# ppwwyyxx/OpenPano

Measured on NVIDIA H100. Metric: Mpixels/sec SIFT+match+blend, higher is better.
Workload: dtype f32

## Files before the change

openpano_b200/csrc/blend.cu:

```cuda
#include "common.cuh"
#include "blend_rows.cuh"
#include "blur_tile.cuh"
#include <math.h>
#include <string.h>
#include <vector>
#include <algorithm>
#include <climits>
#include <memory>

struct BlendImg {
  union {
    const float* rgb;
    const unsigned char* pix;
  };
  int w, h;
  int x0, y0, x1, y1;
  double hi[9];
  long long roi_off;
  long long plane;
  long long mask_off;
  int rw, rh, pitch;
  int channels;
};

// ... 131 lines not shown
  wsum[t] = ws;
}

__global__ void k_linear_resolve(const float* sum, const float* __restrict__ wsum, float* out, size_t n_px, int lazy) {
  const size_t t = (size_t)blockIdx.x * blockDim.x + threadIdx.x;
  if (t >= n_px) return;
  const float* p = sum + t * 3;
  linear_resolve_px(lazy, p[0], p[1], p[2], wsum[t], out + t * 3);
}

template <class Src>
__global__ void k_mb_first_level(const BlendImg* __restrict__ imgs, BlendGeom g, float* __restrict__ cur,
                                 unsigned char* __restrict__ mask) {
  __shared__ float lut[Src::kLut ? 256 : 1];
  if constexpr (Src::kLut) {
    build_rgb8_lut(lut, threadIdx.y * blockDim.x + threadIdx.x);
    __syncthreads();
  }
  const BlendImg& im = imgs[blockIdx.z];
  int j = blockIdx.x * blockDim.x + threadIdx.x;
  int i = blockIdx.y * blockDim.y + threadIdx.y;
  if (j >= im.rw || i >= im.rh) return;
  double x, y;
  coor_func(im, g, j + im.x0, i + im.y0, &x, &y);
  float c0, c1, c2;
  bool ok = interpolate_rgb(blend_src<Src>(im, lut), im.w, im.h, (float)y, (float)x, &c0, &c1, &c2);
  if (ok && fminf(c0, fminf(c1, c2)) < 0) ok = false;
  const size_t o = (size_t)i * im.pitch + j;
  float* p = cur + im.roi_off + o;
  float ww = 0.f;
  if (!ok) { c0 = 0.f; c1 = 0.f; c2 = 0.f; }
  else {
    double ox = x / im.w - 0.5, oy = y / im.h - 0.5;
    double wd = (0.5 - fabs(ox)) * (0.5 - fabs(oy));
    if (wd < 0.0) wd = 0.0;
    ww = (float)(wd + 1e-6);
  }
  p[0] = c0; p[im.plane] = c1; p[2 * im.plane] = c2; p[3 * im.plane] = ww;
  mask[im.mask_off + o] = ok ? 0 : 1;
}

__global__ void k_mb_weight_argmax(const BlendImg* __restrict__ imgs, int n, float* __restrict__ cur, int tw,
                                   int row0, int row1) {
  __shared__ TileList tl;
  {
    const int tj0 = blockIdx.x * blockDim.x, ti0 = row0 + blockIdx.y * blockDim.y;
    build_tile_list(imgs, n, tj0, ti0, tj0 + blockDim.x - 1, ti0 + blockDim.y - 1, &tl);
  }
  int j = blockIdx.x * blockDim.x + threadIdx.x;
  int i = row0 + blockIdx.y * blockDim.y + threadIdx.y;
  if (j >= tw || i >= row1) return;
  const int nl = tl.n < 0 ? n : tl.n;
  float mx = 0.f;
  int best = -1;
  for (int q = 0; q < nl; ++q) {
    const BlendImg& im = imgs[tl.n < 0 ? q : (int)tl.idx[q]];
    if (i >= im.y0 && i <= im.y1 && j >= im.x0 && j <= im.x1) {
      const float w = __ldg(cur + im.roi_off + 3 * im.plane + (size_t)(i - im.y0) * im.pitch + (j - im.x0));
      if (w > mx) { mx = w; best = q; }
    }
  }
  for (int q = 0; q < nl; ++q) {
    const BlendImg& im = imgs[tl.n < 0 ? q : (int)tl.idx[q]];
    if (i >= im.y0 && i <= im.y1 && j >= im.x0 && j <= im.x1)
      cur[im.roi_off + 3 * im.plane + (size_t)(i - im.y0) * im.pitch + (j - im.x0)] = q == best ? 1.f : 0.f;
  }
}

struct BlurTaps { int center; float taps[64]; };
struct MbPlane { long long off; int w, h, pitch, pad; };

template <int C>
__global__ void __launch_bounds__(BT_THREADS, 4)
k_mb_blur_tma(const MbPlane* __restrict__ planes, const int2* __restrict__ span, int n_planes, int n_tiles,
              const TmaDesc* __restrict__ maps, float* __restrict__ dst, const __grid_constant__ BlurTaps bt) {
  extern __shared__ __align__(128) float smem[];
  __shared__ __align__(8) uint64_t s_bar[2];
  __shared__ BlurTile s_tile[2];
  constexpr int RX = (C + 3) & ~3;
  constexpr int GW = BT_W + 2 * RX, GH = BT_H + 2 * C;
  constexpr int GSZ = (GH * GW + 31) & ~31;
  float* grey0 = smem;
  float* colbuf = smem + 2 * GSZ;
  float* outT = colbuf + BLUR_COLBUF_FLOATS(C);
  const int tid = threadIdx.x;
  constexpr uint32_t tile_bytes = (uint32_t)(GH * GW * sizeof(float));
  int t = blockIdx.x;
  if (tid == 0) {
    sbar_init(sm_u32(&s_bar[0]), 1);
    sbar_init(sm_u32(&s_bar[1]), 1);
    asm volatile("fence.mbarrier_init.release.cluster;" ::: "memory");
    if (t < n_tiles) {
      const BlurTile tl = find_blur_tile(span, n_planes, t);
      s_tile[0] = tl;
      sbar_expect_tx(sm_u32(&s_bar[0]), tile_bytes);
      tma_load_2d(sm_u32(grey0), maps + tl.om, tl.tx * BT_W - RX, tl.ty * BT_H - C, sm_u32(&s_bar[0]));
    }
  }
  __syncthreads();
  for (int it = 0; t < n_tiles; t += gridDim.x, ++it) {
    const int b = it & 1;
    float* grey = grey0 + b * GSZ;
    const BlurTile tl = s_tile[b];
    const MbPlane pl = planes[tl.om];
    const int x0 = tl.tx * BT_W, y0 = tl.ty * BT_H;
    if (tid == 0 && t + (int)gridDim.x < n_tiles) {
      const BlurTile nx = find_blur_tile(span, n_planes, t + gridDim.x);
      s_tile[b ^ 1] = nx;
      asm volatile("fence.proxy.async.shared::cta;" ::: "memory");
      sbar_expect_tx(sm_u32(&s_bar[b ^ 1]), tile_bytes);
      tma_load_2d(sm_u32(grey0 + (b ^ 1) * GSZ), maps + nx.om, nx.tx * BT_W - RX, nx.ty * BT_H - C, sm_u32(&s_bar[b ^ 1]));
    }
    sbar_wait(sm_u32(&s_bar[b]), (uint32_t)(it >> 1) & 1u);
    if (x0 - RX < 0 || y0 - C < 0 || x0 + BT_W + RX > pl.w || y0 + BT_H + C > pl.h) {
      for (int i = tid; i < GH * GW; i += BT_THREADS) {
        const int yy = i / GW, xx = i - yy * GW;
        const int gy = y0 + yy - C, gx = x0 + xx - RX;
        const int cy = min(max(gy, 0), pl.h - 1), cx = min(max(gx, 0), pl.w - 1);
        if (cy != gy || cx != gx) grey[i] = grey[(cy - y0 + C) * GW + (cx - x0 + RX)];
      }
      __syncthreads();
    }
    blur_level<C>(grey, colbuf, outT, bt.taps, C, RX, GW, tid);
    const int tx = tid & (BT_W - 1), ty = tid / BT_W;
    const int gx = x0 + tx;
    float* out = dst + pl.off;
#pragma unroll
    for (int i = 0; i < BT_H / 4; ++i) {
      const int y = ty + 4 * i, gy = y0 + y;
      if (gx < pl.w && gy < pl.h) out[(size_t)gy * pl.pitch + gx] = outT[y * (BT_W + 1) + tx];
    }
    __syncthreads();
  }
}

#define MB_TW 64
#define MB_TH 32
__global__ void __launch_bounds__(256)
k_mb_blur_generic(const MbPlane* __restrict__ planes, const int2* __restrict__ span, int n_planes,
                  const float* __restrict__ src, float* __restrict__ dst, const __grid_constant__ BlurTaps bt) {
  extern __shared__ float mb_smem[];
  const BlurTile tl = find_blur_tile(span, n_planes, blockIdx.x);
  const MbPlane pl = planes[tl.om];
  const int tx0 = tl.tx * MB_TW, ty0 = tl.ty * MB_TH;
  const int c = bt.center, kw = 2 * c + 1;
  const int SW = MB_TW + 2 * c, SH = MB_TH + 2 * c;
  float* tile = mb_smem;
  float* colres = mb_smem + SH * SW;
  const float* base = src + pl.off;
  const int tid = threadIdx.x;
  for (int idx = tid; idx < SH * SW; idx += 256) {
    const int r = idx / SW, q = idx - r * SW;
    const int y = min(max(ty0 - c + r, 0), pl.h - 1), x = min(max(tx0 - c + q, 0), pl.w - 1);
    tile[idx] = __ldg(base + (size_t)y * pl.pitch + x);
  }
  __syncthreads();
  for (int idx = tid; idx < MB_TH * SW; idx += 256) {
    const int i = idx / SW, q = idx - i * SW;
    float acc = 0.f;
    const float* col = tile + i * SW + q;
    for (int k = 0; k < kw; ++k) acc += col[k * SW] * bt.taps[k];
    colres[idx] = acc;
  }
  __syncthreads();
  for (int idx = tid; idx < MB_TH * MB_TW; idx += 256) {
    const int i = idx / MB_TW, j = idx - i * MB_TW;
    if (ty0 + i >= pl.h || tx0 + j >= pl.w) continue;
    float acc = 0.f;
    const float* row = colres + i * SW + j;
    for (int k = 0; k < kw; ++k) acc += row[k] * bt.taps[k];
    dst[pl.off + (size_t)(ty0 + i) * pl.pitch + tx0 + j] = acc;
  }
}

__global__ void k_mb_accumulate(const BlendImg* __restrict__ imgs, int n, const float* __restrict__ cur,
                                const float* __restrict__ next, const unsigned char* __restrict__ mask,
                                int first, int is_last, float* __restrict__ out, unsigned char* __restrict__ tmask, int tw,
                                int row0, int row1) {
  __shared__ TileList tl;
  {
    const int tj0 = blockIdx.x * blockDim.x, ti0 = row0 + blockIdx.y * blockDim.y;
    build_tile_list(imgs, n, tj0, ti0, tj0 + blockDim.x - 1, ti0 + blockDim.y - 1, &tl);
  }
  int j = blockIdx.x * blockDim.x + threadIdx.x;
  int i = row0 + blockIdx.y * blockDim.y + threadIdx.y;
  if (j >= tw || i >= row1) return;
  const int nl = tl.n < 0 ? n : tl.n;
  float s0 = 0.f, s1 = 0.f, s2 = 0.f, wsum = 0.f;
  for (int q = 0; q < nl; ++q) {
    const BlendImg& im = imgs[tl.n < 0 ? q : (int)tl.idx[q]];
    if (!(i >= im.y0 && i <= im.y1 && j >= im.x0 && j <= im.x1)) continue;
    const size_t o = (size_t)(i - im.y0) * im.pitch + (j - im.x0);
    const float w = __ldg(cur + im.roi_off + 3 * im.plane + o);
    if (w <= 0) continue;
    if (mask[im.mask_off + o]) continue;
    const float* pc = cur + im.roi_off + o;
    const float c0 = __ldg(pc), c1 = __ldg(pc + im.plane), c2 = __ldg(pc + 2 * im.plane);
    if (!is_last) {
      const float* pn = next + im.roi_off + o;
      const float n0 = __ldg(pn), n1 = __ldg(pn + im.plane), n2 = __ldg(pn + 2 * im.plane);
      s0 += (c0 - n0) * w; s1 += (c1 - n1) * w; s2 += (c2 - n2) * w;
    } else {
      s0 += c0 * w; s1 += c1 * w; s2 += c2 * w;
    }
    wsum += w;
  }
  size_t t = (size_t)(i - row0) * tw + j;
  float* p = out + t * 3;
  bool touched = first ? false : tmask[t] != 0;
  float v0 = -1.f, v1 = -1.f, v2 = -1.f;
  if (touched) { v0 = p[0]; v1 = p[1]; v2 = p[2]; }
  bool dirty = first != 0;
  if (!((double)wsum < 1e-6)) {
    s0 /= wsum; s1 /= wsum; s2 /= wsum;
    if (!touched) { v0 = s0; v1 = s1; v2 = s2; touched = true; }
    else { v0 += s0; v1 += s1; v2 += s2; }
    dirty = true;
  }
  if (is_last && touched) {
    v0 = v0 < 1.0f ? v0 : 1.0f; v0 = v0 > 0.f ? v0 : 0.f;
    v1 = v1 < 1.0f ? v1 : 1.0f; v1 = v1 > 0.f ? v1 : 0.f;
    v2 = v2 < 1.0f ? v2 : 1.0f; v2 = v2 > 0.f ? v2 : 0.f;
    dirty = true;
  }
  if (dirty) { p[0] = v0; p[1] = v1; p[2] = v2; }
  if (first || touched) tmask[t] = touched ? 1 : 0;
}

__global__ void k_fill(float* __restrict__ p, size_t n, float v) {
  size_t i = (size_t)blockIdx.x * blockDim.x + threadIdx.x;
  if (i < n) p[i] = v;
}


struct BlendJob {
  std::vector<BlendImg> imgs;
  std::vector<int> src;
  BlendGeom g;
  int tw = 0, th = 0;
  long long roi_floats = 0;
  long long mask_bytes = 0;
  int max_rw = 0, max_rh = 0;
  std::vector<BlurTaps> level_taps;
  int halo = 0;
  bool strip = false;
  int clip0 = INT_MIN, clip1 = INT_MAX;
  std::vector<double> tab;
  size_t ncol = 0, nrow = 0;
};

struct BlendDev {
  DevBuf<BlendImg> d_imgs;
  DevBuf<double> d_tab;
  DevBuf<float> d_cur, d_next;
  DevBuf<unsigned char> d_mask, d_tmask;
  DevBuf<MbPlane> d_planes;
  DevBuf<int2> d_span;
  DevBuf<TmaDesc> d_maps;
  std::vector<int> centers;
  int n_planes = 0, n_tiles = 0;
  int wrow0 = 0, wrow1 = 0;
};

template <int C>
static cudaError_t launch_mb_blur_tma(pano_ctx* ctx, int grid, const MbPlane* planes, const int2* span, int n_planes,
                                      int n_tiles, const TmaDesc* maps, float* dst, const BlurTaps& bt) {
  constexpr int RX = (C + 3) & ~3, GW = BT_W + 2 * RX, GH = BT_H + 2 * C, GSZ = (GH * GW + 31) & ~31;
  const size_t smem = (size_t)(2 * GSZ + BLUR_COLBUF_FLOATS(C) + BT_H * (BT_W + 1)) * sizeof(float);
  cudaError_t e = cudaFuncSetAttribute(k_mb_blur_tma<C>, cudaFuncAttributeMaxDynamicSharedMemorySize, (int)smem);
  if (e != cudaSuccess) return e;
  k_mb_blur_tma<C><<<grid, BT_THREADS, smem, ctx->stream>>>(planes, span, n_planes, n_tiles, maps, dst, bt);
  return cudaGetLastError();
}

static int level_taps(int bands, int gauss_window_factor, std::vector<BlurTaps>* taps) {
  int halo = 0;
  for (int level = 0; level + 1 < bands; ++level) {
    float sigma = (float)(sqrt(level * 2 + 1.0) * 4);
    BlurTaps bt;
    memset(&bt, 0, sizeof(bt));
    int kw = host_gauss_kernel(sigma, gauss_window_factor, bt.taps, 63);
    if (kw < 0) return kw;
    bt.center = kw / 2;
    halo += bt.center;
    if (taps) taps->push_back(bt);
  }
  return halo;
}

int blend_halo(int bands, const pano_params* p) { return level_taps(bands, p->gauss_window_factor, nullptr); }

static void strip_clip(int bands, int halo, int oh, int row0, int row1, int* clip0, int* clip1) {
  const bool strip = bands > 0 && (row0 != 0 || row1 != oh);
  *clip0 = (strip && row0 > 0) ? std::max(0, row0 - halo) : INT_MIN;
  *clip1 = (strip && row1 < oh) ? row1 + halo - 1 : INT_MAX;
}

bool blend_strip_reads(const pano_blend_image& im, int bands, int halo, int oh, int row0, int row1) {
  if (row0 == 0 && row1 == oh) return true;
  if (bands == 0) return im.y0 < row1 && im.y1 >= row0;
  int c0, c1;
  strip_clip(bands, halo, oh, row0, row1, &c0, &c1);
  return std::max(im.y0, c0) <= std::min(im.y1, c1);
}

static int blend_plan(pano_ctx* ctx, int n, const pano_blend_image* imgs, const pano_blend_geom* g, int bands,
                      const pano_params* p, int ow, int oh, int row0, int row1, bool need_src, BlendJob* job,
                      const unsigned char* const* pix = nullptr, const int* channels = nullptr, bool tables = true) {
  job->halo = level_taps(bands, p->gauss_window_factor, &job->level_taps);
  if (job->halo < 0) return ctx_fail(ctx, PANO_ERR_INVALID, "blend: gaussian window %d too wide", -job->halo);
  job->strip = bands > 0 && (row0 != 0 || row1 != oh);
  strip_clip(bands, job->halo, oh, row0, row1, &job->clip0, &job->clip1);
  job->imgs.reserve(n);
  for (int k = 0; k < n; ++k) {
    const pano_blend_image& s = imgs[k];
    if ((need_src && !s.rgb_hwc) || s.w < 2 || s.h < 2 || s.x1 < s.x0 || s.y1 < s.y0 || s.x0 < 0 || s.y0 < 0)
      return ctx_fail(ctx, PANO_ERR_INVALID, "blend: image %d has an invalid shape or range", k);
    if (pix && !pix[k]) return ctx_fail(ctx, PANO_ERR_INVALID, "blend: image %d has no pixels", k);
    if (pix)
      if (int rc = pix8_check(ctx, "blend", k, channels[k], pix[k])) return rc;
    job->tw = std::max(job->tw, s.x1); job->th = std::max(job->th, s.y1);
    BlendImg d;
    memset(&d, 0, sizeof(d));
    d.rgb = s.rgb_hwc; d.w = s.w; d.h = s.h;
    if (pix) d.pix = pix[k];
    d.x0 = s.x0; d.x1 = s.x1;
    d.y0 = std::max(s.y0, job->clip0); d.y1 = std::min(s.y1, job->clip1);
    if (d.y0 > d.y1) continue;
    memcpy(d.hi, s.homo_inv, sizeof(d.hi));
    d.rw = d.x1 - d.x0 + 1; d.rh = d.y1 - d.y0 + 1;
    d.pitch = (int)align_up((size_t)d.rw, 32);
    d.plane = (long long)d.pitch * d.rh;
    d.roi_off = job->roi_floats;
    d.mask_off = job->mask_bytes;
    d.channels = pix ? channels[k] : 3;
    job->roi_floats += 4 * d.plane;
    job->mask_bytes += d.plane;
    job->max_rw = std::max(job->max_rw, d.rw); job->max_rh = std::max(job->max_rh, d.rh);
    job->imgs.push_back(d);
    job->src.push_back(k);
  }
  if (job->tw != ow || job->th != oh || ow <= 0 || oh <= 0)
    return ctx_fail(ctx, PANO_ERR_INVALID, "blend: output is %dx%d but target_size is %dx%d", ow, oh, job->tw, job->th);
  if (job->imgs.empty()) return PANO_OK;
  job->ncol = (size_t)job->tw + 2; job->nrow = (size_t)job->th + 2;
  if (tables && g->projection != PANO_PROJ_FLAT) {
    job->tab.resize(2 * job->ncol + job->nrow);
    for (size_t j = 0; j < job->ncol; ++j) {
      double cx = (double)j * g->res_x + g->proj_min_x;
      job->tab[j] = sin(cx); job->tab[job->ncol + j] = cos(cx);
    }
// ... 454 lines not shown
```

openpano_b200/csrc/blur_tile.cuh:

```cuda
#pragma once
#include "common.cuh"

#define BT_W 64
#define BT_H 32
#define BT_THREADS 256

struct BlurTile { int om; int tx, ty; };

__device__ __forceinline__ BlurTile find_blur_tile(const int2* __restrict__ span, int n_om, int cta) {
  int lo = 0, hi = n_om - 1;
  while (lo < hi) {
    const int mid = (lo + hi + 1) >> 1;
    if (span[mid].x <= cta) lo = mid; else hi = mid - 1;
  }
  const int local = cta - span[lo].x, tx_n = span[lo].y;
  BlurTile t;
  t.om = lo; t.ty = local / tx_n; t.tx = local - t.ty * tx_n;
  return t;
}

__device__ __forceinline__ float2 fmul2(float2 a, float t) { return make_float2(__fmul_rn(a.x, t), __fmul_rn(a.y, t)); }

#define BLUR_COLBUF_FLOATS(C) (16 * ((((BT_W + 2 * (C) + 2) / 2) * 2) | 1) * 2)

template <int C>
__device__ __forceinline__ void blur_level(const float* __restrict__ grey, float* __restrict__ colbuf,
                                           float* __restrict__ outT, const float* __restrict__ taps_g,
                                           int R, int RX, int GW, int tid) {
  constexpr int KW = 2 * C + 1;
  float tap[KW];
#pragma unroll
  for (int k = 0; k < KW; ++k) tap[k] = taps_g[k];
  const int start = (RX - C) & ~1, off = (RX - C) - start;
  const int npair = (BT_W + 2 * C + off + 1) >> 1;
  const int csp = (2 * npair) | 1;
  float2* colbuf2 = reinterpret_cast<float2*>(colbuf);
  for (int item = tid; item < (BT_H / 8) * npair; item += BT_THREADS) {
    const int strip = item / npair, pr = item - strip * npair;
    const float2* col = reinterpret_cast<const float2*>(grey + (strip * 8 + R - C) * GW + start) + pr;
    const int gw2 = GW >> 1;
    float2 win[8 + 2 * C];
#pragma unroll
    for (int j = 0; j < 8 + 2 * C; ++j) win[j] = col[j * gw2];
#pragma unroll
    for (int r = 0; r < 8; r += 2) {
      float a0x = 0.f, a0y = 0.f, a1x = 0.f, a1y = 0.f;
#pragma unroll
      for (int k = 0; k < KW; ++k) {
        const float2 p0 = fmul2(win[r + k], tap[k]);
        const float2 p1 = fmul2(win[r + 1 + k], tap[k]);
        a0x += p0.x; a0y += p0.y; a1x += p1.x; a1y += p1.y;
      }
      float2* dst = colbuf2 + (strip * 4 + (r >> 1)) * csp + 2 * pr;
      dst[0] = make_float2(a0x, a1x);
      dst[1] = make_float2(a0y, a1y);
    }
  }
  __syncthreads();
  if (tid < 128) {
    const int lane = tid & 31, p = lane & 15, xs = ((tid >> 5) * 2 + (lane >> 4)) * 8;
    const float2* row = colbuf2 + p * csp + off + xs;
    float2 win[8 + 2 * C];
#pragma unroll
    for (int j = 0; j < 8 + 2 * C; ++j) win[j] = row[j];
#pragma unroll
    for (int c = 0; c < 8; ++c) {
      float ax = 0.f, ay = 0.f;
#pragma unroll
      for (int k = 0; k < KW; ++k) {
        const float2 pp = fmul2(win[c + k], tap[k]);
        ax += pp.x; ay += pp.y;
      }
      outT[(2 * p) * (BT_W + 1) + xs + c] = ax;
      outT[(2 * p + 1) * (BT_W + 1) + xs + c] = ay;
    }
  }
  __syncthreads();
}

__device__ __forceinline__ uint32_t sm_u32(const void* p) { return (uint32_t)__cvta_generic_to_shared(p); }
__device__ __forceinline__ void sbar_init(uint32_t bar, uint32_t count) {
  asm volatile("mbarrier.init.shared::cta.b64 [%0], %1;" ::"r"(bar), "r"(count));
}
__device__ __forceinline__ void sbar_expect_tx(uint32_t bar, uint32_t bytes) {
  asm volatile("mbarrier.arrive.expect_tx.shared::cta.b64 _, [%0], %1;" ::"r"(bar), "r"(bytes) : "memory");
}
__device__ __forceinline__ void sbar_wait(uint32_t bar, uint32_t parity) {
  uint32_t done = 0;
  for (uint32_t spin = 0; spin < (1u << 28); ++spin) {
    asm volatile(
        "{\n\t.reg .pred P1;\n\t"
        "mbarrier.try_wait.parity.shared::cta.b64 P1, [%1], %2;\n\t"
        "selp.b32 %0, 1, 0, P1;\n\t}"
        : "=r"(done) : "r"(bar), "r"(parity) : "memory");
    if (done) return;
  }
  __trap();
}
__device__ __forceinline__ void tma_load_2d(uint32_t dst, const TmaDesc* map, int cx, int cy, uint32_t bar) {
  asm volatile("fence.proxy.tensormap::generic.acquire.gpu [%0], 128;" ::"l"(map) : "memory");
  asm volatile(
      "cp.async.bulk.tensor.2d.shared::cluster.global.tile.mbarrier::complete_tx::bytes [%0], [%1, {%2, %3}], [%4];"
      ::"r"(dst), "l"(map), "r"(cx), "r"(cy), "r"(bar) : "memory");
}
```

openpano_b200/csrc/sift.cu:

```cuda
#include "sift.cuh"
#include "desc_interval.h"
#include <math.h>
#include <string.h>
#include <algorithm>
#include <map>
#include <mutex>
#include <cuda.h>

__device__ __forceinline__ void bilinear_coef(int d, float inv, int src_n, int* s, float* frac) {
  float r = ((float)d + 0.5f) * inv - 0.5f;
  int si = (int)floorf(r);
  r -= (float)si;
  if (si < 0) { si = 0; r = 0.f; }
  else if (si + 1 >= src_n) { si = src_n - 2; r = 1.f; }
  *s = si; *frac = r;
}

__device__ __forceinline__ int first_tap_at_least(int t, float inv, int src_n, int dst_n) {
  auto tap = [&](int d) { int s; float f; bilinear_coef(d, inv, src_n, &s, &f); return s; };
  int d = (int)fminf(fmaxf(((float)t + 0.5f) / inv - 0.5f, 0.f), (float)dst_n);
  while (d > 0 && tap(d - 1) >= t) --d;
  while (d < dst_n && tap(d) < t) ++d;
  return d;
}
// ... 105 lines not shown

__device__ __forceinline__ uint32_t make_key(int oct, int scale, int y, int x) {
  return ((uint32_t)oct << 29) | ((uint32_t)scale << 26) | ((uint32_t)y << 13) | (uint32_t)x;
}

template <class DoG>
__device__ __forceinline__ bool is_extremum(float center, float pre_color_thres, float diff_thres, const DoG& dog) {
  if (center < pre_color_thres) return false;
  const float cmp1 = center - diff_thres, cmp2 = center + diff_thres;
  bool mx = true, mn = true;
#pragma unroll
  for (int ds = -1; ds <= 1; ++ds) {
#pragma unroll
    for (int di = -1; di <= 1; ++di)
#pragma unroll
      for (int dj = -1; dj <= 1; ++dj) {
        if (ds == 0 && di == 0 && dj == 0) continue;
        const float v = dog(ds, di, dj);
        if (v >= cmp1) mx = false;
        if (v <= cmp2) mn = false;
      }
    if (!mx && !mn) return false;
  }
  return true;
}

__device__ __forceinline__ void append_candidate(const ExtremaParams& ep, int img, uint32_t key) {
  const int slot = atomicAdd(&ep.cand_count[img], 1);
  if (slot < ep.cap) ep.cand_keys[(size_t)img * ep.cap + slot] = key;
}

#include "blur_tile.cuh"

__global__ void __launch_bounds__(BT_THREADS)
k_blur_dog(const OctMeta* __restrict__ octs, const int2* __restrict__ span, int n_om,
           float* __restrict__ arena, const __grid_constant__ GaussTable gt) {
  extern __shared__ float smem[];
  const BlurTile tl = find_blur_tile(span, n_om, blockIdx.x);
  const OctMeta om = octs[tl.om];
  const int R = gt.rmax;
  const int GW = BT_W + 2 * R;
  const int GH = BT_H + 2 * R;
  float* grey = smem;
  float* colbuf = smem + GH * GW;
  const int x0 = tl.tx * BT_W, y0 = tl.ty * BT_H;
  const float* g0 = arena + om.gauss_off;
  const int tid = threadIdx.x;

  for (int i = tid; i < GH * GW; i += BT_THREADS) {
    int yy = i / GW, xx = i - yy * GW;
    int gy = min(max(y0 + yy - R, 0), om.h - 1);
    int gx = min(max(x0 + xx - R, 0), om.w - 1);
    grey[i] = __ldg(g0 + (size_t)gy * om.pitch + gx);
  }
  __syncthreads();

  const int tx = tid & (BT_W - 1), ty = tid / BT_W;
  for (int s = 0; s < gt.nlev; ++s) {
    const int c = gt.center[s];
    const float* taps = gt.taps[s];
    const int cw = BT_W + 2 * c;
    for (int i = tid; i < BT_H * cw; i += BT_THREADS) {
      int y = i / cw, xx = i - y * cw;
      const float* col = grey + (y + R - c) * GW + (xx + R - c);
      float tmp = 0.f;
      for (int k = 0; k <= 2 * c; ++k) tmp += col[k * GW] * taps[k];
      colbuf[y * GW + xx] = tmp;
    }
    __syncthreads();
    float* lvl = arena + om.gauss_off + (size_t)(s + 1) * om.plane;
#pragma unroll
    for (int i = 0; i < BT_H / 4; ++i) {
      int y = ty + 4 * i;
      const float* row = colbuf + y * GW + tx;
      float tmp = 0.f;
      for (int k = 0; k <= 2 * c; ++k) tmp += row[k] * taps[k];
      int gx = x0 + tx, gy = y0 + y;
      if (gx < om.w && gy < om.h) lvl[(size_t)gy * om.pitch + gx] = tmp;
    }
    __syncthreads();
  }
}

#define EX_RING_FLOATS (3 * BT_H * BT_W)
__global__ void __launch_bounds__(BT_THREADS, 3)
k_blur_extrema(const OctMeta* __restrict__ octs, const int2* __restrict__ span, int n_om, int n_tiles,
               const TmaDesc* __restrict__ maps, float* __restrict__ arena, const __grid_constant__ GaussTable gt,
               const ExtremaParams ep) {
  extern __shared__ __align__(128) float smem[];
  __shared__ __align__(8) uint64_t s_bar[2];
  __shared__ BlurTile s_tile[2];
  const int R = gt.rmax;
  const int RX = (R + 3) & ~3;
  const int GW = BT_W + 2 * RX, GH = BT_H + 2 * R;
  const int GSZ = (GH * GW + 31) & ~31;
  float* grey0 = smem;
  float* colbuf = smem + 2 * GSZ;
  float* outT = colbuf + BLUR_COLBUF_FLOATS(6);
  float* ring = outT + BT_H * (BT_W + 1);
  const int tid = threadIdx.x;
  const uint32_t tile_bytes = (uint32_t)(GH * GW * sizeof(float));
  int t = blockIdx.x;
  if (tid == 0) {
    sbar_init(sm_u32(&s_bar[0]), 1);
    sbar_init(sm_u32(&s_bar[1]), 1);
    asm volatile("fence.mbarrier_init.release.cluster;" ::: "memory");
    if (t < n_tiles) {
      const BlurTile tl = find_blur_tile(span, n_om, t);
      s_tile[0] = tl;
      sbar_expect_tx(sm_u32(&s_bar[0]), tile_bytes);
      tma_load_2d(sm_u32(grey0), maps + tl.om, tl.tx * BT_W - RX, tl.ty * BT_H - R, sm_u32(&s_bar[0]));
    }
  }
  __syncthreads();
  for (int it = 0; t < n_tiles; t += gridDim.x, ++it) {
    const int b = it & 1;
    float* grey = grey0 + b * GSZ;
    const BlurTile tl = s_tile[b];
    const OctMeta om = octs[tl.om];
    const int x0 = tl.tx * BT_W, y0 = tl.ty * BT_H;
    if (tid == 0 && t + (int)gridDim.x < n_tiles) {
      const BlurTile nx = find_blur_tile(span, n_om, t + gridDim.x);
      s_tile[b ^ 1] = nx;
      asm volatile("fence.proxy.async.shared::cta;" ::: "memory");
      sbar_expect_tx(sm_u32(&s_bar[b ^ 1]), tile_bytes);
      tma_load_2d(sm_u32(grey0 + (b ^ 1) * GSZ), maps + nx.om, nx.tx * BT_W - RX, nx.ty * BT_H - R, sm_u32(&s_bar[b ^ 1]));
    }
    sbar_wait(sm_u32(&s_bar[b]), (uint32_t)(it >> 1) & 1u);
    if (x0 - RX < 0 || y0 - R < 0 || x0 + BT_W + RX > om.w || y0 + BT_H + R > om.h) {
      for (int i = tid; i < GH * GW; i += BT_THREADS) {
        const int yy = i / GW, xx = i - yy * GW;
        const int gy = y0 + yy - R, gx = x0 + xx - RX;
        const int cy = min(max(gy, 0), om.h - 1), cx = min(max(gx, 0), om.w - 1);
        if (cy != gy || cx != gx) grey[i] = grey[(cy - y0 + R) * GW + (cx - x0 + RX)];
      }
      __syncthreads();
    }
    const int tx = tid & (BT_W - 1), ty = tid / BT_W;
    const int gx = x0 + tx;
    const bool col_in = gx >= 1 && gx <= om.w - 2;
    const bool col_seam = tx == 0 || tx == BT_W - 1;
    float prev[BT_H / 4];
#pragma unroll
    for (int i = 0; i < BT_H / 4; ++i) prev[i] = grey[(ty + 4 * i + R) * GW + tx + RX];
    for (int s = 0; s < gt.nlev; ++s) {
      if (gt.center[s] == 3) blur_level<3>(grey, colbuf, outT, gt.taps[s], R, RX, GW, tid);
      else blur_level<6>(grey, colbuf, outT, gt.taps[s], R, RX, GW, tid);
      float* lvl = arena + om.gauss_off + (size_t)(s + 1) * om.plane;
      float* dog = ring + (s % 3) * (BT_H * BT_W);
#pragma unroll
      for (int i = 0; i < BT_H / 4; ++i) {
        const int y = ty + 4 * i, gy = y0 + y;
        const float v = outT[y * (BT_W + 1) + tx];
        if (gx < om.w && gy < om.h) lvl[(size_t)gy * om.pitch + gx] = v;
        dog[y * BT_W + tx] = fabsf(prev[i] - v);
        prev[i] = v;
      }
      if (s >= 2) {
        __syncthreads();
        const int j = s - 1;
        const float* d0 = ring + ((s - 2) % 3) * (BT_H * BT_W);
        const float* d1 = ring + ((s - 1) % 3) * (BT_H * BT_W);
        const float* d2 = dog;
#pragma unroll 1
        for (int i = 0; i < BT_H / 4; ++i) {
          const int y = ty + 4 * i, gy = y0 + y;
          if (!col_in || gy < 1 || gy > om.h - 2) continue;
          const int o = y * BT_W + tx;
          const float center = d1[o];
          if (center < ep.pre_color_thres) continue;
          if (col_seam || y == 0 || y == BT_H - 1) {
            const int slot = atomicAdd(&ep.seam_count[om.img], 1);
            if (slot < ep.seam_cap) ep.seam_keys[(size_t)om.img * ep.seam_cap + slot] = make_key(om.oct, j, gy, gx);
            continue;
          }
          auto at = [&](int ds, int di, int dj) {
            const float* d = ds < 0 ? d0 : ds == 0 ? d1 : d2;
            return d[o + di * BT_W + dj];
          };
          if (is_extremum(center, ep.pre_color_thres, ep.diff_thres, at))
            append_candidate(ep, om.img, make_key(om.oct, j, gy, gx));
        }
      }
    }
    __syncthreads();
  }
}

__device__ __forceinline__ void test_from_levels(const ExtremaParams& ep, const OctMeta& om, const float* arena,
                                                 int j, int gy, int gx, float center) {
  const float* c = arena + om.gauss_off + (size_t)gy * om.pitch + gx;
  auto at = [&](int ds, int di, int dj) {
    const float* q = c + (ptrdiff_t)(j + ds) * om.plane + (ptrdiff_t)di * om.pitch + dj;
    return fabsf(__ldg(q) - __ldg(q + om.plane));
  };
  if (is_extremum(center, ep.pre_color_thres, ep.diff_thres, at))
    append_candidate(ep, om.img, make_key(om.oct, j, gy, gx));
}

__global__ void __launch_bounds__(256)
k_extrema_seams(const OctMeta* __restrict__ octs, int n_oct, const float* __restrict__ arena, const ExtremaParams ep) {
  const int img = blockIdx.y;
  const int n = min(ep.seam_count[img], ep.seam_cap);
  for (int i = blockIdx.x * blockDim.x + threadIdx.x; i < n; i += gridDim.x * blockDim.x) {
    const uint32_t key = ep.seam_keys[(size_t)img * ep.seam_cap + i];
    const int oct = key >> 29, j = (key >> 26) & 7, gy = (key >> 13) & 8191, gx = key & 8191;
    const OctMeta om = octs[img * n_oct + oct];
    const float* c = arena + om.gauss_off + (size_t)gy * om.pitch + gx;
    test_from_levels(ep, om, arena, j, gy, gx, fabsf(__ldg(c + (size_t)j * om.plane) - __ldg(c + (size_t)(j + 1) * om.plane)));
  }
}

#define EXS_THREADS 192

__global__ void __launch_bounds__(EXS_THREADS, 6)
k_extrema_scan(const OctMeta* __restrict__ octs, const int2* __restrict__ span, int n_om,
               const float* __restrict__ arena, const ExtremaParams ep) {
  const BlurTile tl = find_blur_tile(span, n_om, blockIdx.x);
  const OctMeta om = octs[tl.om];
  const int x0 = tl.tx * BT_W, y0 = tl.ty * BT_H;
  for (int p = threadIdx.x; p < BT_W * BT_H; p += EXS_THREADS) {
    const int gx = x0 + (p & (BT_W - 1)), gy = y0 + p / BT_W;
    if (gx < 1 || gx > om.w - 2 || gy < 1 || gy > om.h - 2) continue;
    const float* c = arena + om.gauss_off + (size_t)gy * om.pitch + gx;
    float lv[SIFT_MAX_LEVELS];
#pragma unroll
    for (int l = 1; l < SIFT_MAX_LEVELS; ++l) lv[l] = l <= ep.nscale - 2 ? __ldg(c + (size_t)l * om.plane) : 0.f;
#pragma unroll
    for (int j = 1; j < SIFT_MAX_LEVELS - 1; ++j) {
      if (j >= ep.nscale - 2) break;
      test_from_levels(ep, om, arena, j, gy, gx, fabsf(lv[j] - lv[j + 1]));
    }
  }
}

__global__ void __launch_bounds__(256)
k_rank_sort(const int* __restrict__ cand_count, const uint32_t* __restrict__ keys,
            uint32_t* __restrict__ sorted, int cap) {
  __shared__ uint32_t sk[1024];
  const int img = blockIdx.y;
  const int n = min(cand_count[img], cap);
  const uint32_t* k = keys + (size_t)img * cap;
  for (int c0 = blockIdx.x * 256; c0 < n; c0 += gridDim.x * 256) {
    const int i = c0 + threadIdx.x;
    uint32_t mine = i < n ? k[i] : 0xffffffffu;
// ... 758 lines not shown
      }
    }
    plan->fast = true;
    for (int s = 0; s < gt.nlev; ++s) plan->fast = plan->fast && (gt.center[s] == 3 || gt.center[s] == 6);
    const int R = gt.rmax;
    if (((size_t)(BT_H + 2 * R) * (BT_W + 2 * R) + (size_t)BT_H * (BT_W + 2 * R)) * sizeof(float) > 200 * 1024)
      return ctx_fail(ctx, PANO_ERR_INVALID, "sift: blur halo too large");

    const size_t nlist = (size_t)n * cap;
    if (int rc = plan_alloc(ctx, plan.get(), wk->arena, off)) return rc;
    if (int rc = plan_alloc(ctx, plan.get(), wk->d_img, n)) return rc;
    if (int rc = plan_alloc(ctx, plan.get(), wk->d_oct, wk->h_oct.size())) return rc;
    if (int rc = plan_alloc(ctx, plan.get(), wk->d_maps, (size_t)n * n_oct)) return rc;
    if (int rc = plan_alloc(ctx, plan.get(), wk->d_tilespan, tilespan.size())) return rc;
    if (int rc = plan_alloc(ctx, plan.get(), wk->cand_count, 2 * n + 2)) return rc;
    if (int rc = plan_alloc(ctx, plan.get(), wk->seam_keys, (size_t)n * seam_cap)) return rc;
    if (int rc = plan_alloc(ctx, plan.get(), wk->cand_keys, nlist)) return rc;
    if (int rc = plan_alloc(ctx, plan.get(), wk->sorted_keys, nlist)) return rc;
    if (int rc = plan_alloc(ctx, plan.get(), wk->refined, nlist)) return rc;
    if (int rc = plan_alloc(ctx, plan.get(), wk->kp_valid, nlist)) return rc;
    if (int rc = plan_alloc(ctx, plan.get(), wk->npeaks, nlist)) return rc;
    if (int rc = plan_alloc(ctx, plan.get(), wk->dirs, nlist * SIFT_MAX_PEAKS)) return rc;
    if (int rc = plan_alloc(ctx, plan.get(), wk->n_refined, n)) return rc;
    if (int rc = plan_alloc(ctx, plan.get(), wk->desc_cand, nlist)) return rc;
    if (int rc = plan_alloc(ctx, plan.get(), wk->desc_dir, nlist)) return rc;
  }
  SiftWork* wk = plan->wk.get();
  const GaussTable& gt = plan->gt;
  const bool fast = plan->fast;
  const size_t seam_cap = plan->seam_cap;
  for (int i = 0; i < n; ++i) {
    if (channels) wk->h_img[i].pix = (const unsigned char*)d_src[i];
    else wk->h_img[i].src = (const float*)d_src[i];
  }

  const size_t nlist = (size_t)n * cap;
  const int n_om = n * n_oct;
  fs->ctx = ctx; fs->n_images = n; fs->cap = cap;
  if (int rc = fs->d_desc.alloc(ctx, nlist * 128)) return rc;
  if (int rc = fs->d_coor.alloc(ctx, nlist * 4)) return rc;
  fs->d_real = fs->d_coor + nlist * 2;
  if (int rc = fs->d_count.alloc(ctx, n)) return rc;
  fs->base.resize(n);
  for (int i = 0; i < n; ++i) fs->base[i] = (long long)i * cap;

  {
    void* dsts[4] = {wk->d_img, wk->cand_count, wk->d_oct, wk->d_tilespan};
    const void* srcs[4] = {wk->h_img.data(), nullptr, wk->h_oct.data(), tilespan.data()};
    size_t sizes[4] = {n * sizeof(ImgMeta), (2 * n + 2) * sizeof(int), wk->h_oct.size() * sizeof(OctMeta),
                       tilespan.size() * sizeof(int2)};
    if (int rc = ctx_put_many(ctx, fresh ? 4 : 2, dsts, srcs, sizes)) return rc;
  }
  if (fresh && fast) {
    std::vector<TmaDesc> maps(n_om);
    const int R = gt.rmax;
    for (int k = 0; k < n_om; ++k) {
      const OctMeta& om = wk->h_oct[k];
      unsigned long long dims[2] = {(unsigned long long)om.w, (unsigned long long)om.h};
      unsigned long long strides[1] = {(unsigned long long)om.pitch * sizeof(float)};
      unsigned box[2] = {(unsigned)(BT_W + 2 * ((R + 3) & ~3)), (unsigned)(BT_H + 2 * R)};
      if (int rc = ctx_tma_encode(ctx, &maps[k], wk->arena + om.gauss_off, 2, dims, strides, box)) return rc;
    }
    if (int rc = ctx_put(ctx, wk->d_maps, maps.data(), maps.size() * sizeof(TmaDesc))) return rc;
  }

  {
    dim3 g(ceil_div(plan->max_w0, PG_TW), ceil_div(plan->max_h0, PG_TH), n);
    float* work = keep ? wk->arena.get() : nullptr;
    if (channels && std::any_of(channels, channels + n, pix8_layout))
      PANO_LAUNCH(ctx, "k_pyramid_grey_pix8", k_pyramid_grey<SrcPix8>, g, PG_THREADS, 0, wk->d_img, wk->d_oct, n_oct, wk->arena, work);
    else if (channels)
      PANO_LAUNCH(ctx, "k_pyramid_grey_rgb8", k_pyramid_grey<SrcRgb8>, g, PG_THREADS, 0, wk->d_img, wk->d_oct, n_oct, wk->arena, work);
    else
      PANO_LAUNCH(ctx, "k_pyramid_grey", k_pyramid_grey<SrcF32>, g, PG_THREADS, 0, wk->d_img, wk->d_oct, n_oct, wk->arena, work);
  }
  {
    const ExtremaParams ep{n_scale, p->pre_color_thres, p->judge_extrema_diff_thres, cap, wk->cand_count, wk->cand_keys,
                           (int)seam_cap, wk->cand_count + n + 2, wk->seam_keys};
    const int R = gt.rmax;
    size_t smem = ((size_t)(BT_H + 2 * R) * (BT_W + 2 * R) + (size_t)BT_H * (BT_W + 2 * R)) * sizeof(float);
    if (fast) {
      const int GW = BT_W + 2 * ((R + 3) & ~3), GH = BT_H + 2 * R;
      const size_t gsz = ((size_t)GH * GW + 31) & ~(size_t)31;
      size_t smf = (2 * gsz + (size_t)BLUR_COLBUF_FLOATS(6) + (size_t)BT_H * (BT_W + 1) + EX_RING_FLOATS) * sizeof(float);
      PANO_CUDA(ctx, sift_smem_limit(ctx, (const void*)k_blur_extrema, smf));
      const int grid = std::min(wk->n_tiles, ctx->num_sms * 3);
      PANO_LAUNCH(ctx, "k_blur_extrema", k_blur_extrema, grid, BT_THREADS, smf, wk->d_oct, wk->d_tilespan, n_om, wk->n_tiles,
                  wk->d_maps, wk->arena, gt, ep);
      PANO_LAUNCH(ctx, "k_extrema_seams", k_extrema_seams, dim3(8, n), 256, 0, wk->d_oct, n_oct, wk->arena, ep);
    } else {
      if (smem > 48 * 1024)
        PANO_CUDA(ctx, sift_smem_limit(ctx, (const void*)k_blur_dog, smem));
      PANO_LAUNCH(ctx, "k_blur_dog_generic", k_blur_dog, wk->n_tiles, BT_THREADS, smem, wk->d_oct, wk->d_tilespan, n_om, wk->arena, gt);
      PANO_LAUNCH(ctx, "k_extrema_scan", k_extrema_scan, wk->n_tiles, EXS_THREADS, 0, wk->d_oct, wk->d_tilespan, n_om,
                  wk->arena, ep);
    }
  }
  {
    dim3 g(8, n);
    PANO_LAUNCH(ctx, "k_rank_sort", k_rank_sort, g, 256, 0, wk->cand_count, wk->cand_keys, wk->sorted_keys, cap);
    RefineParams rp{n_scale, p->calc_offset_depth, p->offset_thres, p->contrast_thres, p->edge_ratio,
                    p->gauss_sigma, p->scale_factor};
    dim3 g4(16, n);
    PANO_LAUNCH(ctx, "k_refine", k_refine, g4, 128, 0, wk->d_oct, wk->arena, n_oct, wk->cand_count, wk->sorted_keys, rp, cap,
                wk->refined, wk->kp_valid);
    PANO_LAUNCH(ctx, "k_orientation", k_orientation, ctx->num_sms * 8, ORI_WARPS * 32, 0, wk->d_oct, wk->arena, n_oct, n, cap,
                wk->cand_count, wk->refined, wk->kp_valid, p->ori_radius, p->ori_hist_smooth_count, wk->npeaks, wk->dirs,
                wk->cand_count + n + 1);
    PANO_LAUNCH(ctx, "k_expand_scan", k_expand_scan, n, SCAN_THREADS, 0, wk->cand_count, wk->kp_valid, wk->npeaks,
                wk->dirs, cap, fs->d_count, wk->n_refined, wk->desc_cand, wk->desc_dir);
    DescParams dp{p->desc_hist_scale_factor, p->desc_int_factor};
    const size_t dsm = sizeof(DescQuadSmem) * DESC_WARPS;
    PANO_CUDA(ctx, sift_smem_limit(ctx, (const void*)k_descriptor, dsm));
    const int grid = ctx->num_sms * DESC_MIN_CTAS;
    PANO_LAUNCH(ctx, "k_descriptor", k_descriptor, grid, DESC_THREADS, dsm, wk->d_oct, wk->d_img, wk->arena, n_oct, n, cap,
                wk->refined, fs->d_count, wk->desc_cand, wk->desc_dir, dp, fs->d_desc, fs->d_coor, wk->cand_count + n);
  }
  wk->n_desc = fs->d_count;

  if (!fs->h_count_pinned.get()) {
    fs->h_count_pinned = ctx_small_pinned_get(ctx, (size_t)2 * n * sizeof(int) + 16);
    if (!fs->h_count_pinned.get()) return ctx_fail(ctx, PANO_ERR_CUDA, "pinned allocation failed");
  }
  {
    int* h_counts = (int*)fs->h_count_pinned.get();
    void* dsts[2] = {h_counts, h_counts + n};
    const void* srcs[2] = {fs->d_count, wk->cand_count};
    size_t sizes[2] = {n * sizeof(int), n * sizeof(int)};
    if (int rc = ctx_store_many(ctx, 2, dsts, srcs, sizes)) return rc;
  }
  PANO_CUDA(ctx, ctx_signal(ctx, &fs->counts_token));
  fs->counts_pending = true;
  fs->counts_on_host = false;

  if (keep) {
    *keep = std::move(plan->wk);
  } else if (ctx->cache_limit && plan->bytes <= ctx->cache_limit) {
    ctx->sift_plan = std::move(plan);
    if (ctx->cached_bytes + ctx->sift_plan->bytes > ctx->cache_limit) ctx_cache_release(ctx, ctx->cache_limit - ctx->sift_plan->bytes);
  }
  return PANO_OK;
}


int featureset_sync_counts(pano_featureset* fs) {
  SlowCall sc("featureset_sync_counts");
  if (fs->error) return fs->error;
  if (fs->counts_on_host) return PANO_OK;
  pano_ctx* ctx = fs->ctx;
  while (fs->counts_pending) {
    cudaError_t e = ctx_wait_signal(ctx, fs->counts_token);
    if (e != cudaSuccess) return fs->error = ctx_cuda(ctx, e, "feature count read-back");
    fs->counts_pending = false;
    const int n = fs->n_images;
    const int* h_counts = (const int*)fs->h_count_pinned.get();
    int worst = 0;
    for (int i = 0; i < n; ++i) worst = std::max(worst, std::max(h_counts[i], h_counts[n + i]));
    if (worst <= fs->cap) {
      fs->h_count.assign(h_counts, h_counts + n);
      break;
    }
    int cap = fs->cap;
    while (cap < worst && cap < SIFT_CAP_MAX) cap *= 2;
    if (cap < worst || fs->src.empty())
      return fs->error = ctx_fail(ctx, PANO_ERR_CAPACITY, "sift: %d list entries in one image exceed the capacity %d", worst, fs->cap);
    fs->d_desc.reset(); fs->d_coor.reset(); fs->d_count.reset();
    fs->d_real = nullptr;
// ... 12 lines not shown
```

Before: 11140.

## Replace block-wide separable blur with per-warp band blur and vector stores

Reworks the separable Gaussian blur so each warp owns a 4-row band: the vertical pass writes into a private, XOR-swizzled band buffer and each lane then produces 8 contiguous horizontal outputs. This removes the two block-wide __syncthreads and the transposed outT staging buffer, and lets results be written with float4 stores to global memory and the DoG ring. The DoG ring grows to 4 slots, presumably so the next level's ring writes cannot race with the extremum scan without a barrier. The cost is more shared memory for the ring, more registers for the 8-output windows, and some redundant vertical work on the partial column round.

```diff
diff --git a/openpano_b200/csrc/blend.cu b/openpano_b200/csrc/blend.cu
--- a/openpano_b200/csrc/blend.cu
+++ b/openpano_b200/csrc/blend.cu
@@ -237,7 +237,6 @@
   constexpr int GSZ = (GH * GW + 31) & ~31;
   float* grey0 = smem;
   float* colbuf = smem + 2 * GSZ;
-  float* outT = colbuf + BLUR_COLBUF_FLOATS(C);
   const int tid = threadIdx.x;
   constexpr uint32_t tile_bytes = (uint32_t)(GH * GW * sizeof(float));
   int t = blockIdx.x;
@@ -276,14 +275,20 @@
       }
       __syncthreads();
     }
-    blur_level<C>(grey, colbuf, outT, bt.taps, C, RX, GW, tid);
-    const int tx = tid & (BT_W - 1), ty = tid / BT_W;
-    const int gx = x0 + tx;
-    float* out = dst + pl.off;
+    const int warp = tid >> 5, lane = tid & 31;
+    float v[8];
+    blur_band<C>(grey, colbuf + warp * (BAND_ROWS * BAND_STRIDE(C)), bt.taps, C, RX, GW, warp, lane, v);
+    const int gy = y0 + BAND_ROWS * warp + (lane >> 3), gx = x0 + 8 * (lane & 7);
+    if (gy < pl.h) {
+      float* p = dst + pl.off + (size_t)gy * pl.pitch + gx;
+      if (gx + 8 <= pl.w) {
+        reinterpret_cast<float4*>(p)[0] = make_float4(v[0], v[1], v[2], v[3]);
+        reinterpret_cast<float4*>(p)[1] = make_float4(v[4], v[5], v[6], v[7]);
+      } else {
 #pragma unroll
-    for (int i = 0; i < BT_H / 4; ++i) {
-      const int y = ty + 4 * i, gy = y0 + y;
-      if (gx < pl.w && gy < pl.h) out[(size_t)gy * pl.pitch + gx] = outT[y * (BT_W + 1) + tx];
+        for (int i = 0; i < 8; ++i)
+          if (gx + i < pl.w) p[i] = v[i];
+      }
     }
     __syncthreads();
   }
@@ -421,7 +426,7 @@
 static cudaError_t launch_mb_blur_tma(pano_ctx* ctx, int grid, const MbPlane* planes, const int2* span, int n_planes,
                                       int n_tiles, const TmaDesc* maps, float* dst, const BlurTaps& bt) {
   constexpr int RX = (C + 3) & ~3, GW = BT_W + 2 * RX, GH = BT_H + 2 * C, GSZ = (GH * GW + 31) & ~31;
-  const size_t smem = (size_t)(2 * GSZ + BLUR_COLBUF_FLOATS(C) + BT_H * (BT_W + 1)) * sizeof(float);
+  const size_t smem = (size_t)(2 * GSZ + BLUR_COLBUF_FLOATS(C)) * sizeof(float);
   cudaError_t e = cudaFuncSetAttribute(k_mb_blur_tma<C>, cudaFuncAttributeMaxDynamicSharedMemorySize, (int)smem);
   if (e != cudaSuccess) return e;
   k_mb_blur_tma<C><<<grid, BT_THREADS, smem, ctx->stream>>>(planes, span, n_planes, n_tiles, maps, dst, bt);
diff --git a/openpano_b200/csrc/blur_tile.cuh b/openpano_b200/csrc/blur_tile.cuh
--- a/openpano_b200/csrc/blur_tile.cuh
+++ b/openpano_b200/csrc/blur_tile.cuh
@@ -19,63 +19,75 @@
   return t;
 }
 
-__device__ __forceinline__ float2 fmul2(float2 a, float t) { return make_float2(__fmul_rn(a.x, t), __fmul_rn(a.y, t)); }
-
-#define BLUR_COLBUF_FLOATS(C) (16 * ((((BT_W + 2 * (C) + 2) / 2) * 2) | 1) * 2)
+#define BAND_ROWS 4
+#define BAND_STRIDE(C) ((BT_W + 2 * (C) + 7) & ~7)
+#define BLUR_COLBUF_FLOATS(C) (BT_H * BAND_STRIDE(C))
 
 template <int C>
-__device__ __forceinline__ void blur_level(const float* __restrict__ grey, float* __restrict__ colbuf,
-                                           float* __restrict__ outT, const float* __restrict__ taps_g,
-                                           int R, int RX, int GW, int tid) {
-  constexpr int KW = 2 * C + 1;
+__device__ __forceinline__ void blur_band(const float* __restrict__ grey, float* __restrict__ band,
+                                          const float* __restrict__ taps_g, int R, int RX, int GW,
+                                          int warp, int lane, float (&out)[8]) {
+  constexpr int KW = 2 * C + 1, NC = BT_W + 2 * C, RS = BAND_STRIDE(C);
+  constexpr int NW = 8 + 2 * C, NB = (NW + 7) / 8;
+  static_assert(BT_H == BAND_ROWS * (BT_THREADS / 32), "one 4-row band per warp");
   float tap[KW];
 #pragma unroll
   for (int k = 0; k < KW; ++k) tap[k] = taps_g[k];
-  const int start = (RX - C) & ~1, off = (RX - C) - start;
-  const int npair = (BT_W + 2 * C + off + 1) >> 1;
-  const int csp = (2 * npair) | 1;
-  float2* colbuf2 = reinterpret_cast<float2*>(colbuf);
-  for (int item = tid; item < (BT_H / 8) * npair; item += BT_THREADS) {
-    const int strip = item / npair, pr = item - strip * npair;
-    const float2* col = reinterpret_cast<const float2*>(grey + (strip * 8 + R - C) * GW + start) + pr;
-    const int gw2 = GW >> 1;
-    float2 win[8 + 2 * C];
+  __syncwarp();
+  constexpr int NF = BT_W / 32, NP = NC - 32 * NF;
+  constexpr int G = NP * 4 <= 32 ? 4 : NP * 2 <= 32 ? 2 : 1, RPG = BAND_ROWS / G;
+  static_assert(NF == 2 && NP > 0 && NP <= 32, "64 + 2C columns: two full rounds and one partial");
+  const float* g = grey + (BAND_ROWS * warp + R - C) * GW + (RX - C);
 #pragma unroll
-    for (int j = 0; j < 8 + 2 * C; ++j) win[j] = col[j * gw2];
+  for (int q = 0; q < NF; ++q) {
+    float win[BAND_ROWS + 2 * C];
 #pragma unroll
-    for (int r = 0; r < 8; r += 2) {
-      float a0x = 0.f, a0y = 0.f, a1x = 0.f, a1y = 0.f;
+    for (int i = 0; i < BAND_ROWS + 2 * C; ++i) win[i] = g[i * GW + 32 * q + lane];
+    float* dst = band + 32 * q + (lane ^ ((q & 1) << 2));
 #pragma unroll
-      for (int k = 0; k < KW; ++k) {
-        const float2 p0 = fmul2(win[r + k], tap[k]);
-        const float2 p1 = fmul2(win[r + 1 + k], tap[k]);
-        a0x += p0.x; a0y += p0.y; a1x += p1.x; a1y += p1.y;
-      }
-      float2* dst = colbuf2 + (strip * 4 + (r >> 1)) * csp + 2 * pr;
-      dst[0] = make_float2(a0x, a1x);
-      dst[1] = make_float2(a0y, a1y);
+    for (int r = 0; r < BAND_ROWS; ++r) {
+      float acc = 0.f;
+#pragma unroll
+      for (int k = 0; k < KW; ++k) acc += __fmul_rn(win[r + k], tap[k]);
+      dst[r * RS] = acc;
     }
   }
-  __syncthreads();
-  if (tid < 128) {
-    const int lane = tid & 31, p = lane & 15, xs = ((tid >> 5) * 2 + (lane >> 4)) * 8;
-    const float2* row = colbuf2 + p * csp + off + xs;
-    float2 win[8 + 2 * C];
+  if (lane < G * NP) {
+    const int grp = lane / NP, c = 32 * NF + (lane - grp * NP);
+    constexpr int NWIN = G * (RPG - 1) + 1 + 2 * C;
+    float win[NWIN];
 #pragma unroll
-    for (int j = 0; j < 8 + 2 * C; ++j) win[j] = row[j];
+    for (int i = 0; i < NWIN; ++i) win[i] = g[(grp + i) * GW + c];
+    float* dst = band + grp * RS + c;
 #pragma unroll
-    for (int c = 0; c < 8; ++c) {
-      float ax = 0.f, ay = 0.f;
+    for (int r = 0; r < RPG; ++r) {
+      float acc = 0.f;
 #pragma unroll
-      for (int k = 0; k < KW; ++k) {
-        const float2 pp = fmul2(win[c + k], tap[k]);
-        ax += pp.x; ay += pp.y;
-      }
-      outT[(2 * p) * (BT_W + 1) + xs + c] = ax;
-      outT[(2 * p + 1) * (BT_W + 1) + xs + c] = ay;
+      for (int k = 0; k < KW; ++k) acc += __fmul_rn(win[G * r + k], tap[k]);
+      dst[G * r * RS] = acc;
     }
   }
-  __syncthreads();
+  __syncwarp();
+  const int r = lane >> 3, b = lane & 7;
+  float win[8 * NB];
+#pragma unroll
+  for (int m = 0; m < NB; ++m) {
+    const int t = b + m, sw = t & 4;
+    const float* blk = band + r * RS + 8 * t;
+    const float4 lo = *reinterpret_cast<const float4*>(blk + sw);
+    win[8 * m] = lo.x; win[8 * m + 1] = lo.y; win[8 * m + 2] = lo.z; win[8 * m + 3] = lo.w;
+    if (8 * m + 4 < NW) {
+      const float4 hi = *reinterpret_cast<const float4*>(blk + (sw ^ 4));
+      win[8 * m + 4] = hi.x; win[8 * m + 5] = hi.y; win[8 * m + 6] = hi.z; win[8 * m + 7] = hi.w;
+    }
+  }
+#pragma unroll
+  for (int c = 0; c < 8; ++c) {
+    float acc = 0.f;
+#pragma unroll
+    for (int k = 0; k < KW; ++k) acc += __fmul_rn(win[c + k], tap[k]);
+    out[c] = acc;
+  }
 }
 
 __device__ __forceinline__ uint32_t sm_u32(const void* p) { return (uint32_t)__cvta_generic_to_shared(p); }
diff --git a/openpano_b200/csrc/sift.cu b/openpano_b200/csrc/sift.cu
--- a/openpano_b200/csrc/sift.cu
+++ b/openpano_b200/csrc/sift.cu
@@ -211,7 +211,8 @@
   }
 }
 
-#define EX_RING_FLOATS (3 * BT_H * BT_W)
+#define EX_RING_SLOTS 4
+#define EX_RING_FLOATS (EX_RING_SLOTS * BT_H * BT_W)
 __global__ void __launch_bounds__(BT_THREADS, 3)
 k_blur_extrema(const OctMeta* __restrict__ octs, const int2* __restrict__ span, int n_om, int n_tiles,
                const TmaDesc* __restrict__ maps, float* __restrict__ arena, const __grid_constant__ GaussTable gt,
@@ -225,8 +226,7 @@
   const int GSZ = (GH * GW + 31) & ~31;
   float* grey0 = smem;
   float* colbuf = smem + 2 * GSZ;
-  float* outT = colbuf + BLUR_COLBUF_FLOATS(6);
-  float* ring = outT + BT_H * (BT_W + 1);
+  float* ring = colbuf + BLUR_COLBUF_FLOATS(6);
   const int tid = threadIdx.x;
   const uint32_t tile_bytes = (uint32_t)(GH * GW * sizeof(float));
   int t = blockIdx.x;
@@ -269,27 +269,45 @@
     const int gx = x0 + tx;
     const bool col_in = gx >= 1 && gx <= om.w - 2;
     const bool col_seam = tx == 0 || tx == BT_W - 1;
-    float prev[BT_H / 4];
-#pragma unroll
-    for (int i = 0; i < BT_H / 4; ++i) prev[i] = grey[(ty + 4 * i + R) * GW + tx + RX];
+    const int warp = tid >> 5, lane = tid & 31;
+    float* band = colbuf + warp * (BAND_ROWS * BAND_STRIDE(6));
+    const int by = BAND_ROWS * warp + (lane >> 3), bx = 8 * (lane & 7);
+    const int bgy = y0 + by, bgx = x0 + bx;
+    float prev[8];
+    {
+      const float* gp = grey + (by + R) * GW + RX + bx;
+      const float4 a = *reinterpret_cast<const float4*>(gp), c = *reinterpret_cast<const float4*>(gp + 4);
+      prev[0] = a.x; prev[1] = a.y; prev[2] = a.z; prev[3] = a.w;
+      prev[4] = c.x; prev[5] = c.y; prev[6] = c.z; prev[7] = c.w;
+    }
     for (int s = 0; s < gt.nlev; ++s) {
-      if (gt.center[s] == 3) blur_level<3>(grey, colbuf, outT, gt.taps[s], R, RX, GW, tid);
-      else blur_level<6>(grey, colbuf, outT, gt.taps[s], R, RX, GW, tid);
-      float* lvl = arena + om.gauss_off + (size_t)(s + 1) * om.plane;
-      float* dog = ring + (s % 3) * (BT_H * BT_W);
-#pragma unroll
-      for (int i = 0; i < BT_H / 4; ++i) {
-        const int y = ty + 4 * i, gy = y0 + y;
-        const float v = outT[y * (BT_W + 1) + tx];
-        if (gx < om.w && gy < om.h) lvl[(size_t)gy * om.pitch + gx] = v;
-        dog[y * BT_W + tx] = fabsf(prev[i] - v);
-        prev[i] = v;
-      }
+      float v[8];
+      if (gt.center[s] == 3) blur_band<3>(grey, band, gt.taps[s], R, RX, GW, warp, lane, v);
+      else blur_band<6>(grey, band, gt.taps[s], R, RX, GW, warp, lane, v);
+      if (bgy < om.h) {
+        float* p = arena + om.gauss_off + (size_t)(s + 1) * om.plane + (size_t)bgy * om.pitch + bgx;
+        if (bgx + 8 <= om.w) {
+          reinterpret_cast<float4*>(p)[0] = make_float4(v[0], v[1], v[2], v[3]);
+          reinterpret_cast<float4*>(p)[1] = make_float4(v[4], v[5], v[6], v[7]);
+        } else {
+#pragma unroll
+          for (int i = 0; i < 8; ++i)
+            if (bgx + i < om.w) p[i] = v[i];
+        }
+      }
+      float* dog = ring + (s % EX_RING_SLOTS) * (BT_H * BT_W);
+      float* dp = dog + by * BT_W + bx;
+      reinterpret_cast<float4*>(dp)[0] = make_float4(fabsf(prev[0] - v[0]), fabsf(prev[1] - v[1]),
+                                                     fabsf(prev[2] - v[2]), fabsf(prev[3] - v[3]));
+      reinterpret_cast<float4*>(dp)[1] = make_float4(fabsf(prev[4] - v[4]), fabsf(prev[5] - v[5]),
+                                                     fabsf(prev[6] - v[6]), fabsf(prev[7] - v[7]));
+#pragma unroll
+      for (int i = 0; i < 8; ++i) prev[i] = v[i];
       if (s >= 2) {
         __syncthreads();
         const int j = s - 1;
-        const float* d0 = ring + ((s - 2) % 3) * (BT_H * BT_W);
-        const float* d1 = ring + ((s - 1) % 3) * (BT_H * BT_W);
+        const float* d0 = ring + ((s - 2) % EX_RING_SLOTS) * (BT_H * BT_W);
+        const float* d1 = ring + ((s - 1) % EX_RING_SLOTS) * (BT_H * BT_W);
         const float* d2 = dog;
 #pragma unroll 1
         for (int i = 0; i < BT_H / 4; ++i) {
@@ -1214,7 +1232,7 @@
     if (fast) {
       const int GW = BT_W + 2 * ((R + 3) & ~3), GH = BT_H + 2 * R;
       const size_t gsz = ((size_t)GH * GW + 31) & ~(size_t)31;
-      size_t smf = (2 * gsz + (size_t)BLUR_COLBUF_FLOATS(6) + (size_t)BT_H * (BT_W + 1) + EX_RING_FLOATS) * sizeof(float);
+      size_t smf = (2 * gsz + (size_t)BLUR_COLBUF_FLOATS(6) + EX_RING_FLOATS) * sizeof(float);
       PANO_CUDA(ctx, sift_smem_limit(ctx, (const void*)k_blur_extrema, smf));
       const int grid = std::min(wk->n_tiles, ctx->num_sms * 3);
       PANO_LAUNCH(ctx, "k_blur_extrema", k_blur_extrema, grid, BT_THREADS, smf, wk->d_oct, wk->d_tilespan, n_om, wk->n_tiles,
```

New measurement: 11320 (median of 6 runs). No clear change (+1.7%).
